# soedinglab/spacedust

Hardware: AMD Instinct MI355X
Metric: clustersearch throughput (genome-pairs/s; SW GCUPS alongside) (higher is better)
Workload: dtype int16

## Files before the change

spacedust_amd/csrc/hip/sd_sw_pk.h:

```cpp
#ifndef SD_SW_PK_H
#define SD_SW_PK_H

#include <hip/hip_runtime.h>
#include <cstdint>

namespace sdpk {

struct SwTask {
    uint64_t qOff;
    uint64_t tOff;
    int32_t n;
    int32_t tL;
    int32_t qStep;
    int32_t tStep;
    int32_t segLen;
    uint32_t slot;
    uint64_t boundOff;
};

typedef short s16x2 __attribute__((ext_vector_type(2)));
typedef unsigned short u16x2 __attribute__((ext_vector_type(2)));

__device__ __forceinline__ uint32_t pkMax(uint32_t a, uint32_t b) {
    return __builtin_bit_cast(uint32_t, __builtin_elementwise_max(__builtin_bit_cast(s16x2, a), __builtin_bit_cast(s16x2, b)));
}
__device__ __forceinline__ uint32_t pkSubSat(uint32_t a, uint32_t b) {
    return __builtin_bit_cast(uint32_t, __builtin_elementwise_sub_sat(__builtin_bit_cast(u16x2, a), __builtin_bit_cast(u16x2, b)));
}
__device__ __forceinline__ uint32_t pkSub(uint32_t a, uint32_t b) {
    return __builtin_bit_cast(uint32_t, (s16x2) (__builtin_bit_cast(s16x2, a) - __builtin_bit_cast(s16x2, b)));
}
__device__ __forceinline__ uint32_t pkAdd(uint32_t a, uint32_t b) {
    return __builtin_bit_cast(uint32_t, (s16x2) (__builtin_bit_cast(s16x2, a) + __builtin_bit_cast(s16x2, b)));
}
__device__ __forceinline__ uint32_t pkLshr(uint32_t a, int s) {
    return __builtin_bit_cast(uint32_t, (u16x2) (__builtin_bit_cast(u16x2, a) >> (u16x2) ((unsigned short) s)));
}
__device__ __forceinline__ uint32_t pkAshr(uint32_t a, int s) {
    return __builtin_bit_cast(uint32_t, (s16x2) (__builtin_bit_cast(s16x2, a) >> (s16x2) ((short) s)));
}
__device__ __forceinline__ uint32_t pkRowCode(uint32_t g, int code) {
    uint32_t r;
    asm("v_pk_mad_i16 %0, %1, 32, %2 op_sel_hi:[1,0,0] clamp" : "=v"(r) : "v"(g), "s"(code));
    return r;
}
__device__ __forceinline__ uint32_t bfi(uint32_t mask, uint32_t a, uint32_t b) { return (a & mask) | (b & ~mask); }

__device__ __forceinline__ void addProfile4(uint32_t pa, uint32_t pb, uint32_t d0, uint32_t d1, uint32_t d2, uint32_t d3,
                                            uint32_t &h0, uint32_t &h1, uint32_t &h2, uint32_t &h3) {
    asm("v_add_u16_sdwa %0, %4, sext(%8) dst_sel:WORD_0 dst_unused:UNUSED_PAD src0_sel:WORD_0 src1_sel:BYTE_0\n\t"
        "v_add_u16_sdwa %1, %5, sext(%8) dst_sel:WORD_0 dst_unused:UNUSED_PAD src0_sel:WORD_0 src1_sel:BYTE_1\n\t"
        "v_add_u16_sdwa %2, %6, sext(%8) dst_sel:WORD_0 dst_unused:UNUSED_PAD src0_sel:WORD_0 src1_sel:BYTE_2\n\t"
        "v_add_u16_sdwa %3, %7, sext(%8) dst_sel:WORD_0 dst_unused:UNUSED_PAD src0_sel:WORD_0 src1_sel:BYTE_3\n\t"
        "v_add_u16_sdwa %0, %4, sext(%9) dst_sel:WORD_1 dst_unused:UNUSED_PRESERVE src0_sel:WORD_1 src1_sel:BYTE_0\n\t"
        "v_add_u16_sdwa %1, %5, sext(%9) dst_sel:WORD_1 dst_unused:UNUSED_PRESERVE src0_sel:WORD_1 src1_sel:BYTE_1\n\t"
        "v_add_u16_sdwa %2, %6, sext(%9) dst_sel:WORD_1 dst_unused:UNUSED_PRESERVE src0_sel:WORD_1 src1_sel:BYTE_2\n\t"
        "v_add_u16_sdwa %3, %7, sext(%9) dst_sel:WORD_1 dst_unused:UNUSED_PRESERVE src0_sel:WORD_1 src1_sel:BYTE_3\n\t"
        "s_nop 0"
        : "=&v"(h0), "=&v"(h1), "=&v"(h2), "=&v"(h3)
        : "v"(d0), "v"(d1), "v"(d2), "v"(d3), "v"(pa), "v"(pb));
}

__device__ __forceinline__ uint32_t dppShr1(uint32_t v) {
    return (uint32_t) __builtin_amdgcn_update_dpp(0, (int) v, 0x138 , 0xf, 0xf, false);
}

template <int LANE>
__device__ __forceinline__ uint32_t writeLane(uint32_t value, uint32_t old) {
    asm("v_writelane_b32 %0, %1, %2" : "+v"(old) : "s"(value), "n"(LANE));
    return old;
}
__device__ __forceinline__ uint32_t readLane(uint32_t v, int lane) {
#if defined(__HIP_DEVICE_COMPILE__)
    return (uint32_t) __builtin_amdgcn_readlane((int) v, lane);
#else
    (void) lane;
    return v;
#endif
}

constexpr int PK_NEUTRAL = 21;

template <int RT, int LW, bool MULTI, bool WIDE, bool SHARED>
__global__ void __launch_bounds__(64)
sw_score_pk_kernel(const SwTask *__restrict__ tasks, uint32_t nTasks, const uint8_t *__restrict__ qRes,
                   const int8_t *__restrict__ qBias, const uint8_t *__restrict__ tRes, const int8_t *__restrict__ mat,
                   int go, int ge, int32_t *__restrict__ out, uint2 *__restrict__ boundary,
                   const uint32_t *__restrict__ order,
                   const int8_t *__restrict__ qProf ) {
    constexpr int ROWS = LW * RT;
    constexpr int WORDS = (RT + 3) / 4;
    constexpr int RTP = 4 * WORDS;
    constexpr int PSTRIDE = LW * WORDS;
    constexpr int NGRP = 64 / LW;
    constexpr int NT = 2 * NGRP;
    __shared__ uint32_t prof[SHARED ? NGRP : NT][22][PSTRIDE];
    __shared__ int8_t smat[441];
    for (int i = threadIdx.x; i < 441; i += 64) smat[i] = mat[i];
    __syncthreads();

    const int lane = threadIdx.x;
    const int grp = lane / LW, l = lane % LW;
    SwTask tk[NT];
#pragma unroll
    for (int x = 0; x < NT; x++) {
        const uint32_t id = blockIdx.x * NT + x;
        const uint32_t tid = id < nTasks ? (order ? order[id] : id) : 0xFFFFFFFFu;
        if (tid != 0xFFFFFFFFu) {
            tk[x] = tasks[tid];
        } else {
            tk[x].n = 0; tk[x].tL = 0; tk[x].qOff = 0; tk[x].tOff = 0; tk[x].qStep = 1; tk[x].tStep = 1; tk[x].segLen = 1;
            tk[x].slot = 0; tk[x].boundOff = 0;
        }
    }
    const SwTask A = (NGRP == 2 && grp) ? tk[NT - 2] : tk[0];
    SwTask B = (NGRP == 2 && grp) ? tk[NT - 1] : tk[1];
    const bool haveA = A.n > 0, haveB = B.n > 0;
    if (SHARED && !haveB) {
        B = A;
        B.tL = 0;
    }
    int maxN = 0, maxTL = 0;
#pragma unroll
    for (int x = 0; x < NT; x++) {
        maxN = max(maxN, tk[x].n);
        maxTL = max(maxTL, tk[x].tL);
    }
    const int pairTL = max(A.tL, B.tL);
    const int nStrips = MULTI ? (maxN + ROWS - 1) / ROWS : (maxN > 0 ? 1 : 0);
    const int steps = (maxN > 0 && maxTL > 0) ? maxTL + LW - 1 : 0;
    uint4 *bnd = nullptr;
    if (MULTI) bnd = (uint4 *) (boundary + (A.tL >= B.tL ? A.boundOff : B.boundOff));

    const uint32_t goP = (uint32_t) go | ((uint32_t) go << 16), geP = (uint32_t) ge | ((uint32_t) ge << 16);
    unsigned long long keyA = 0, keyB = 0;
    const uint32_t *profA = &prof[SHARED ? grp : 2 * grp][0][0] + l * WORDS;
    const uint32_t *profB = SHARED ? profA : &prof[2 * grp + 1][0][0] + l * WORDS;

    for (int strip = 0; strip < nStrips; strip++) {
        const int q0 = strip * ROWS + l * RT;
        uint32_t mask[RTP];
        if (strip > 0) __syncthreads();
#pragma unroll
        for (int x = 0; x < (SHARED ? 1 : 2); x++) {
            const SwTask &T = x ? B : A;
            uint32_t *pw = &prof[SHARED ? grp : 2 * grp + x][0][0] + l * WORDS;
            int seg = T.segLen > 0 ? q0 % T.segLen : 0;
#pragma unroll
            for (int w = 0; w < WORDS; w++) {
                int res[4], cb[4];
                int64_t pidx[4];
                bool valid[4];
#pragma unroll
                for (int b = 0; b < 4; b++) {
                    const int qi = q0 + 4 * w + b;
                    valid[b] = (4 * w + b < RT) && qi < T.n;
                    res[b] = 20;
                    cb[b] = 0;
                    pidx[b] = 0;
                    if (valid[b]) {
                        const int64_t idx = (int64_t) T.qOff + (int64_t) qi * T.qStep;
                        res[b] = qRes[idx];
                        cb[b] = qBias[idx];
                        pidx[b] = idx * 21;
                    }
                    const bool reset = valid[b] && seg == 0;
                    seg = (seg + 1 == T.segLen) ? 0 : seg + 1;
                    const uint32_t m = reset ? 0u : 0xFFFFu;
                    if (SHARED) mask[4 * w + b] = m | (m << 16);
                    else if (x == 0) mask[4 * w + b] = m;
                    else mask[4 * w + b] |= m << 16;
                }
                if (qProf) {
                    for (int a = 0; a < 21; a++) {
                        uint32_t word = 0;
#pragma unroll
                        for (int b = 0; b < 4; b++) {
                            const int v = valid[b] ? (int) qProf[pidx[b] + a] : -64;
                            word |= (uint32_t) (uint8_t) (int8_t) v << (8 * b);
                        }
                        pw[a * PSTRIDE + w] = word;
                    }
                } else {
                    for (int a = 0; a < 21; a++) {
                        uint32_t word = 0;
#pragma unroll
                        for (int b = 0; b < 4; b++) {
                            const int v = valid[b] ? (int) smat[a * 21 + res[b]] + cb[b] : -64;
                            word |= (uint32_t) (uint8_t) (int8_t) v << (8 * b);
                        }
                        pw[a * PSTRIDE + w] = word;
                    }
                }
                pw[PK_NEUTRAL * PSTRIDE + w] = 0xC0C0C0C0u;
            }
        }
        __syncthreads();

        uint32_t H[RTP], E[RTP];
#pragma unroll
        for (int r = 0; r < RTP; r++) {
            H[r] = 0;
            E[r] = 0;
        }
        uint32_t outG = 0, outFf = 0, outFl = 0, prevInG = 0;
        uint32_t curT = PK_NEUTRAL | (PK_NEUTRAL << 8);
        uint32_t bestv = 0, bestcm = 0, bestcol = 0;
        uint32_t bestA = 0, bestB = 0, bcolA = 0, bcolB = 0;
        uint32_t ccol = (uint32_t) (-l) & 0xFFFFu;
        ccol |= ccol << 16;
        const bool lastStrip = strip == nStrips - 1;
        const bool readBound = MULTI && strip > 0;

        auto loadChunk = [&](int c0) -> uint32_t {
            const int col = c0 + l;
            uint32_t a = PK_NEUTRAL, b = PK_NEUTRAL;
            if (col < A.tL) a = tRes[(int64_t) A.tOff + (int64_t) col * A.tStep];
            if (col < B.tL) b = tRes[(int64_t) B.tOff + (int64_t) col * B.tStep];
            return a | (b << 8);
        };
        auto loadBound = [&](int c0) -> uint4 {
            const int col = c0 + l;
            uint4 v = make_uint4(0, 0, 0, 0);
            if (readBound && col < pairTL) {
                const unsigned long long lo = __hip_atomic_load((unsigned long long *) &bnd[col], __ATOMIC_RELAXED, __HIP_MEMORY_SCOPE_AGENT);
                const unsigned long long hi = __hip_atomic_load((unsigned long long *) &bnd[col] + 1, __ATOMIC_RELAXED, __HIP_MEMORY_SCOPE_AGENT);
                v.x = (uint32_t) lo; v.y = (uint32_t) (lo >> 32); v.z = (uint32_t) hi;
            }
            return v;
        };
        if (readBound) __threadfence();

        uint32_t chunk = loadChunk(0);
        uint4 bchunk = loadBound(0);
        for (int k0 = 0; k0 < steps; k0 += LW) {
            const uint32_t chunkNext = loadChunk(k0 + LW);
            uint4 bnext = make_uint4(0, 0, 0, 0);
            if (readBound) bnext = loadBound(k0 + LW);
            const int iEnd = min(LW, steps - k0);
#pragma unroll 1
            for (int i = 0; i < iEnd; i++) {
                uint32_t inT = dppShr1(curT), inG = dppShr1(outG), inFf = dppShr1(outFf), inFl = dppShr1(outFl);
                inT = writeLane<0>(readLane(chunk, i), inT);
                if (NGRP == 2) inT = writeLane<32>(readLane(chunk, 32 + i), inT);
                if (readBound) {
                    inG = writeLane<0>(readLane(bchunk.x, i), inG);
                    inFf = writeLane<0>(readLane(bchunk.y, i), inFf);
                    inFl = writeLane<0>(readLane(bchunk.z, i), inFl);
                    if (NGRP == 2) {
                        inG = writeLane<32>(readLane(bchunk.x, 32 + i), inG);
                        inFf = writeLane<32>(readLane(bchunk.y, 32 + i), inFf);
                        inFl = writeLane<32>(readLane(bchunk.z, 32 + i), inFl);
                    }
                } else if (NGRP == 2) {
                    inG = writeLane<32>(0, inG);
                    inFf = writeLane<32>(0, inFf);
                    inFl = writeLane<32>(0, inFl);
                }
                curT = inT;
                const uint32_t *pa = profA + (curT & 0xFFu) * PSTRIDE;
                const uint32_t *pb = profB + (curT >> 8) * PSTRIDE;
                uint32_t h[RTP];
#pragma unroll
                for (int w = 0; w < WORDS; w++) {
                    const uint32_t d0 = (w == 0) ? prevInG : H[4 * w - 1];
                    addProfile4(pa[w], pb[w], d0, H[4 * w], H[4 * w + 1], H[4 * w + 2], h[4 * w], h[4 * w + 1], h[4 * w + 2],
                                h[4 * w + 3]);
                }
                prevInG = inG;
                uint32_t Fl = inFl, Ff = inFf, cm = 0, cmA = 0, cmB = 0;
#pragma unroll
                for (int r = 0; r < RT; r++) {
                    Fl &= mask[r];
                    const uint32_t hpre = pkMax(pkMax(h[r], E[r]), Fl);
                    const uint32_t g = pkMax(hpre, Ff);
                    const uint32_t open = pkSubSat(hpre, goP);
                    E[r] = pkMax(pkSubSat(E[r], geP), open);
                    Fl = pkMax(pkSubSat(Fl, geP), open);
                    Ff = pkMax(pkSubSat(Ff, geP), open);
                    H[r] = g;
                    if (WIDE) {
                        cmA = max(cmA, (g << 16) | (uint32_t) (31 - r));
                        cmB = max(cmB, (g & 0xFFFF0000u) | (uint32_t) (31 - r));
                    } else {
                        cm = pkMax(cm, pkRowCode(g, 31 - r));
                    }
                }
                outG = H[RT - 1];
                outFf = Ff;
                outFl = Fl;
                if (MULTI && !lastStrip && l == LW - 1) {
                    const int c = k0 + i - (LW - 1);
                    if (c >= 0 && c < pairTL) {
                        const unsigned long long lo = (unsigned long long) outG | ((unsigned long long) outFf << 32);
                        __hip_atomic_store((unsigned long long *) &bnd[c], lo, __ATOMIC_RELAXED, __HIP_MEMORY_SCOPE_AGENT);
                        __hip_atomic_store((unsigned long long *) &bnd[c] + 1, (unsigned long long) outFl, __ATOMIC_RELAXED,
                                           __HIP_MEMORY_SCOPE_AGENT);
                    }
                }
                if (WIDE) {
                    const bool upA = cmA > (bestA | 0xFFFFu), upB = cmB > (bestB | 0xFFFFu);
                    bestA = upA ? cmA : bestA;
                    bcolA = upA ? ccol : bcolA;
                    bestB = upB ? cmB : bestB;
                    bcolB = upB ? ccol : bcolB;
                } else {
                    const uint32_t v = pkLshr(cm, 5);
                    const uint32_t nb = pkMax(bestv, v);
                    const uint32_t m = pkAshr(pkSub(bestv, nb), 15);
                    bestcm = bfi(m, cm, bestcm);
                    bestcol = bfi(m, ccol, bestcol);
                    bestv = nb;
                }
                ccol = pkAdd(ccol, 0x00010001u);
            }
            chunk = chunkNext;
            bchunk = bnext;
        }
        {
            const uint32_t vA = WIDE ? bestA >> 16 : bestv & 0xFFFFu, vB = WIDE ? bestB >> 16 : bestv >> 16;
            const uint32_t rcA = WIDE ? bestA & 31u : bestcm & 31u, rcB = WIDE ? bestB & 31u : (bestcm >> 16) & 31u;
            const uint32_t rowA = (uint32_t) (q0 + 31 - (int) rcA), rowB = (uint32_t) (q0 + 31 - (int) rcB);
            const uint32_t colA = WIDE ? bcolA & 0xFFFFu : bestcol & 0xFFFFu, colB = WIDE ? bcolB >> 16 : bestcol >> 16;
            if (vA > 0) {
                const unsigned long long kk = ((unsigned long long) vA << 40) | ((unsigned long long) (0xFFFFFu - colA) << 20) |
                                              (unsigned long long) (0xFFFFFu - rowA);
                keyA = kk > keyA ? kk : keyA;
            }
            if (vB > 0) {
                const unsigned long long kk = ((unsigned long long) vB << 40) | ((unsigned long long) (0xFFFFFu - colB) << 20) |
                                              (unsigned long long) (0xFFFFFu - rowB);
                keyB = kk > keyB ? kk : keyB;
            }
        }
    }
#pragma unroll
    for (int off = LW / 2; off >= 1; off >>= 1) {
        const unsigned long long oa = __shfl_xor(keyA, off, LW), ob = __shfl_xor(keyB, off, LW);
        keyA = oa > keyA ? oa : keyA;
        keyB = ob > keyB ? ob : keyB;
    }
    if (l == 0) {
        if (haveA) {
            const int v = (int) (keyA >> 40);
            out[3 * A.slot + 0] = v;
            out[3 * A.slot + 1] = v == 0 ? -1 : 0xFFFFF - (int) ((keyA >> 20) & 0xFFFFF);
            out[3 * A.slot + 2] = v == 0 ? A.n - 1 : 0xFFFFF - (int) (keyA & 0xFFFFF);
        }
        if (haveB) {
            const int v = (int) (keyB >> 40);
            out[3 * B.slot + 0] = v;
            out[3 * B.slot + 1] = v == 0 ? -1 : 0xFFFFF - (int) ((keyB >> 20) & 0xFFFFF);
            out[3 * B.slot + 2] = v == 0 ? B.n - 1 : 0xFFFFF - (int) (keyB & 0xFFFFF);
        }
    }
}

__device__ __forceinline__ uint32_t pkAshr15(uint32_t a) {
    uint32_t r;
    asm("v_pk_ashrrev_i16 %0, 15, %1 op_sel_hi:[0,1]" : "=v"(r) : "v"(a));
    return r;
}
__device__ __forceinline__ uint32_t bfiAsm(uint32_t mask, uint32_t a, uint32_t b) {
    uint32_t r;
    asm("v_bfi_b32 %0, %1, %2, %3" : "=v"(r) : "v"(mask), "v"(a), "v"(b));
    return r;
}
__device__ __forceinline__ uint32_t addWord0(uint32_t base, uint32_t packed) {
    uint32_t r;
    asm("v_add_u32_sdwa %0, %1, %2 dst_sel:DWORD dst_unused:UNUSED_PAD src0_sel:DWORD src1_sel:WORD_0" : "=v"(r) : "v"(base), "v"(packed));
    return r;
}
__device__ __forceinline__ uint32_t addWord1(uint32_t base, uint32_t packed) {
    uint32_t r;
    asm("v_add_u32_sdwa %0, %1, %2 dst_sel:DWORD dst_unused:UNUSED_PAD src0_sel:DWORD src1_sel:WORD_1" : "=v"(r) : "v"(base), "v"(packed));
    return r;
}

template <int RT, bool SHARED>
__global__ void __launch_bounds__(64)
sw_score_pk_aligned_kernel(const SwTask *__restrict__ tasks, uint32_t nTasks, const uint8_t *__restrict__ qRes,
                           const int8_t *__restrict__ qBias, const uint8_t *__restrict__ tRes, const int8_t *__restrict__ mat,
                           int go, int ge, int32_t *__restrict__ out, const uint32_t *__restrict__ order,
                           const int8_t *__restrict__ qProf) {
    constexpr int LW = 32;
    constexpr int WORDS = (RT + 3) / 4;
    constexpr int RTP = 4 * WORDS;
    constexpr int PSTRIDE = LW * WORDS;
    constexpr int NGRP = 64 / LW;
    constexpr int NT = 2 * NGRP;
    constexpr uint32_t ROWB = PSTRIDE * 4;
    static_assert(22 * ROWB < 65536, "row offsets travel in 16 bits");
    __shared__ uint32_t prof[SHARED ? 1 : NT][22][PSTRIDE];
    __shared__ int8_t smat[441];
    for (int i = threadIdx.x; i < 441; i += 64) smat[i] = mat[i];
    __syncthreads();
    const int lane = threadIdx.x & 63, wave = threadIdx.x >> 6;
    const int grp = lane / LW, l = lane % LW;
    SwTask tk[NT];
#pragma unroll
    for (int x = 0; x < NT; x++) {
        const uint32_t id = (blockIdx.x + (uint32_t) wave) * NT + x;
        const uint32_t tid = id < nTasks ? (order ? order[id] : id) : 0xFFFFFFFFu;
        if (tid != 0xFFFFFFFFu) {
            tk[x] = tasks[tid];
        } else {
            tk[x].n = 0; tk[x].tL = 0; tk[x].qOff = 0; tk[x].tOff = 0; tk[x].qStep = 1; tk[x].tStep = 1; tk[x].segLen = 1;
            tk[x].slot = 0; tk[x].boundOff = 0;
        }
    }
    SwTask A = tk[0], B = tk[1];
#pragma unroll
    for (int g = 1; g < NGRP; g++)
        if (grp == g) {
            A = tk[2 * g];
            B = tk[2 * g + 1];
        }
    const bool haveA = A.n > 0, haveB = B.n > 0;
    if (SHARED && !haveB) {
        B = A;
        B.tL = 0;
    }
    int maxN = 0, maxTL = 0;
#pragma unroll
    for (int x = 0; x < NT; x++) {
        maxN = max(maxN, tk[x].n);
        maxTL = max(maxTL, tk[x].tL);
    }
    const int steps = (maxN > 0 && maxTL > 0) ? maxTL + LW - 1 : 0;
    const uint32_t goP = (uint32_t) go | ((uint32_t) go << 16), geP = (uint32_t) ge | ((uint32_t) ge << 16);
    const int q0 = l * RT;
#pragma unroll
    for (int x = 0; x < (SHARED ? 1 : 2); x++) {
        const SwTask &T = SHARED ? tk[0] : (x ? B : A);
        uint32_t *pw = &prof[SHARED ? 0 : 2 * grp + x][0][0] + l * WORDS;
#pragma unroll
        for (int w = 0; w < WORDS; w++) {
            int res[4], cb[4];
            int64_t pidx[4];
            bool valid[4];
#pragma unroll
            for (int b = 0; b < 4; b++) {
                const int qi = q0 + 4 * w + b;
                valid[b] = (4 * w + b < RT) && qi < T.n;
                res[b] = 20;
                cb[b] = 0;
                pidx[b] = 0;
                if (valid[b]) {
                    const int64_t idx = (int64_t) T.qOff + (int64_t) qi * T.qStep;
                    res[b] = qRes[idx];
                    cb[b] = qBias[idx];
                    pidx[b] = idx * 21;
                }
            }
            const int aFirst = SHARED ? wave * NGRP + grp : 0, aStep = SHARED ? NGRP : 1;
            if (qProf) {
                for (int a = aFirst; a < 21; a += aStep) {
                    uint32_t word = 0;
#pragma unroll
                    for (int b = 0; b < 4; b++) {
                        const int v = valid[b] ? (int) qProf[pidx[b] + a] : -64;
                        word |= (uint32_t) (uint8_t) (int8_t) v << (8 * b);
                    }
                    pw[a * PSTRIDE + w] = word;
                }
            } else {
                for (int a = aFirst; a < 21; a += aStep) {
                    uint32_t word = 0;
#pragma unroll
                    for (int b = 0; b < 4; b++) {
                        const int v = valid[b] ? (int) smat[a * 21 + res[b]] + cb[b] : -64;
                        word |= (uint32_t) (uint8_t) (int8_t) v << (8 * b);
                    }
                    pw[a * PSTRIDE + w] = word;
                }
            }
            pw[PK_NEUTRAL * PSTRIDE + w] = 0xC0C0C0C0u;
        }
    }
    __syncthreads();
    typedef __attribute__((address_space(3))) uint32_t lds_u32;
    const uint32_t baseA = (uint32_t) (size_t) (lds_u32 *) (&prof[SHARED ? 0 : 2 * grp][0][0] + l * WORDS);
    const uint32_t baseB = SHARED ? baseA : (uint32_t) (size_t) (lds_u32 *) (&prof[2 * grp + 1][0][0] + l * WORDS);
    auto ldsWord = [](uint32_t addr, int w) -> uint32_t { return *((const lds_u32 *) (size_t) addr + w); };

    uint32_t H[RTP], E[RTP];
#pragma unroll
    for (int r = 0; r < RTP; r++) {
        H[r] = 0;
        E[r] = 0;
    }
    uint32_t outG = 0, outFf = 0, prevInG = 0;
    uint32_t bestcm = 0, bestcol = 0;
    constexpr uint32_t NEUT = (uint32_t) PK_NEUTRAL * ROWB;
    auto loadChunk = [&](int c0) -> uint32_t {
        const int col = c0 + l;
        uint32_t a = PK_NEUTRAL, b = PK_NEUTRAL;
        if (col < A.tL) a = tRes[(int64_t) A.tOff + (int64_t) col * A.tStep];
        if (col < B.tL) b = tRes[(int64_t) B.tOff + (int64_t) col * B.tStep];
        return (a * ROWB) | ((b * ROWB) << 16);
    };
    uint32_t chunk = loadChunk(0);
    uint32_t chunkNext = loadChunk(LW);
    uint32_t T = NEUT | (NEUT << 16);
    T = writeLane<0>(readLane(chunk, 0), T);
    T = writeLane<32>(readLane(chunk, 32), T);
    uint32_t pa[WORDS], pb[WORDS];
    {
        const uint32_t aA = addWord0(baseA, T), aB = addWord1(baseB, T);
#pragma unroll
        for (int w = 0; w < WORDS; w++) {
            pa[w] = ldsWord(aA, w);
            pb[w] = ldsWord(aB, w);
        }
    }
    auto columnStep = [&](const int k, const uint32_t &Tc, const uint32_t (&pac)[WORDS], const uint32_t (&pbc)[WORDS], uint32_t &Tn,
                          uint32_t (&pan)[WORDS], uint32_t (&pbn)[WORDS]) {
        const int i1 = (k + 1) & (LW - 1);
        if (i1 == 0) {
            chunk = chunkNext;
            chunkNext = loadChunk(k + 1 + LW);
        }
        Tn = dppShr1(Tc);
        Tn = writeLane<0>(readLane(chunk, i1), Tn);
        Tn = writeLane<32>(readLane(chunk, 32 + i1), Tn);
        {
            const uint32_t aA = addWord0(baseA, Tn), aB = addWord1(baseB, Tn);
#pragma unroll
            for (int w = 0; w < WORDS; w++) {
                pan[w] = ldsWord(aA, w);
                pbn[w] = ldsWord(aB, w);
            }
        }
        uint32_t inG = dppShr1(outG), inFf = dppShr1(outFf);
        inG = writeLane<32>(0, inG);
        inFf = writeLane<32>(0, inFf);
        uint32_t h[RTP];
#pragma unroll
        for (int w = 0; w < WORDS; w++) {
            const uint32_t d0 = (w == 0) ? prevInG : H[4 * w - 1];
            addProfile4(pac[w], pbc[w], d0, H[4 * w], H[4 * w + 1], H[4 * w + 2], h[4 * w], h[4 * w + 1], h[4 * w + 2], h[4 * w + 3]);
        }
        prevInG = inG;
        uint32_t Fl = 0, Ff = inFf, cm = 0;
#pragma unroll
        for (int r = 0; r < RT; r++) {
            uint32_t hpre = pkMax(h[r], E[r]);
            if (r != 0) hpre = pkMax(hpre, Fl);
            const uint32_t g = pkMax(hpre, Ff);
            const uint32_t open = pkSubSat(hpre, goP);
            E[r] = pkMax(pkSubSat(E[r], geP), open);
            if (r == 0) Fl = open;
            else if (r + 1 != RT) Fl = pkMax(pkSubSat(Fl, geP), open);
            Ff = pkMax(pkSubSat(Ff, geP), open);
            H[r] = g;
            const uint32_t code = pkRowCode(g, 31 - r);
            cm = r == 0 ? code : pkMax(cm, code);
        }
        outG = H[RT - 1];
        outFf = Ff;
        const uint32_t t = bestcm | 0x001F001Fu;
        const uint32_t m = pkAshr15(pkSub(t, cm));
        const uint32_t kk = (uint32_t) k | ((uint32_t) k << 16);
        bestcm = bfiAsm(m, cm, bestcm);
        bestcol = bfiAsm(m, kk, bestcol);
    };
    uint32_t T2, pa2[WORDS], pb2[WORDS];
#pragma unroll 1
    for (int k = 0; k < steps; k += 2) {
        columnStep(k, T, pa, pb, T2, pa2, pb2);
        columnStep(k + 1, T2, pa2, pb2, T, pa, pb);
    }
    unsigned long long keyA = 0, keyB = 0;
    {
        const uint32_t vA = (bestcm & 0xFFFFu) >> 5, vB = bestcm >> 21;
        const uint32_t rowA = (uint32_t) (q0 + 31 - (int) (bestcm & 31u)), rowB = (uint32_t) (q0 + 31 - (int) ((bestcm >> 16) & 31u));
        const uint32_t colA = (bestcol & 0xFFFFu) - (uint32_t) l, colB = (bestcol >> 16) - (uint32_t) l;
        if (vA > 0) keyA = ((unsigned long long) vA << 40) | ((unsigned long long) (0xFFFFFu - colA) << 20) | (unsigned long long) (0xFFFFFu - rowA);
        if (vB > 0) keyB = ((unsigned long long) vB << 40) | ((unsigned long long) (0xFFFFFu - colB) << 20) | (unsigned long long) (0xFFFFFu - rowB);
    }
#pragma unroll
    for (int off = LW / 2; off >= 1; off >>= 1) {
        const unsigned long long oa = __shfl_xor(keyA, off, LW), ob = __shfl_xor(keyB, off, LW);
        keyA = oa > keyA ? oa : keyA;
        keyB = ob > keyB ? ob : keyB;
    }
    if (l == 0) {
        if (haveA) {
            const int v = (int) (keyA >> 40);
            out[3 * A.slot + 0] = v;
            out[3 * A.slot + 1] = v == 0 ? -1 : 0xFFFFF - (int) ((keyA >> 20) & 0xFFFFF);
            out[3 * A.slot + 2] = v == 0 ? A.n - 1 : 0xFFFFF - (int) (keyA & 0xFFFFF);
        }
        if (haveB) {
            const int v = (int) (keyB >> 40);
            out[3 * B.slot + 0] = v;
            out[3 * B.slot + 1] = v == 0 ? -1 : 0xFFFFF - (int) ((keyB >> 20) & 0xFFFFF);
            out[3 * B.slot + 2] = v == 0 ? B.n - 1 : 0xFFFFF - (int) (keyB & 0xFFFFF);
        }
    }
}

}
#endif
```

Baseline: 2628.

## Software-pipeline profile LDS loads and restructure F-chain in packed SW kernels

In the general packed kernel, target residues are pre-scaled to LDS byte offsets, and the profile words for the next column are loaded one step ahead. This uses a double-buffered two-step loop with SDWA address adds, replacing the per-column pointer arithmetic and dependent loads. Chunk and boundary reloads are folded into the column step at 32-column boundaries. In the aligned kernel, the far-F chain is rewritten as a decaying carry plus a final max with Fl, which shortens the per-row dependency work. The change adds register pressure from the extra profile buffers and reorders the F recurrence, which could alter results if it is not exactly equivalent.

After: 2671, median of 6. No clear change (+1.6%).

```diff
diff --git a/spacedust_amd/csrc/hip/sd_sw_pk.h b/spacedust_amd/csrc/hip/sd_sw_pk.h
--- a/spacedust_amd/csrc/hip/sd_sw_pk.h
+++ b/spacedust_amd/csrc/hip/sd_sw_pk.h
@@ -79,6 +79,27 @@
 #endif
 }
 
+__device__ __forceinline__ uint32_t pkAshr15(uint32_t a) {
+    uint32_t r;
+    asm("v_pk_ashrrev_i16 %0, 15, %1 op_sel_hi:[0,1]" : "=v"(r) : "v"(a));
+    return r;
+}
+__device__ __forceinline__ uint32_t bfiAsm(uint32_t mask, uint32_t a, uint32_t b) {
+    uint32_t r;
+    asm("v_bfi_b32 %0, %1, %2, %3" : "=v"(r) : "v"(mask), "v"(a), "v"(b));
+    return r;
+}
+__device__ __forceinline__ uint32_t addWord0(uint32_t base, uint32_t packed) {
+    uint32_t r;
+    asm("v_add_u32_sdwa %0, %1, %2 dst_sel:DWORD dst_unused:UNUSED_PAD src0_sel:DWORD src1_sel:WORD_0" : "=v"(r) : "v"(base), "v"(packed));
+    return r;
+}
+__device__ __forceinline__ uint32_t addWord1(uint32_t base, uint32_t packed) {
+    uint32_t r;
+    asm("v_add_u32_sdwa %0, %1, %2 dst_sel:DWORD dst_unused:UNUSED_PAD src0_sel:DWORD src1_sel:WORD_1" : "=v"(r) : "v"(base), "v"(packed));
+    return r;
+}
+
 constexpr int PK_NEUTRAL = 21;
 
 template <int RT, int LW, bool MULTI, bool WIDE, bool SHARED>
@@ -94,6 +115,8 @@
     constexpr int PSTRIDE = LW * WORDS;
     constexpr int NGRP = 64 / LW;
     constexpr int NT = 2 * NGRP;
+    constexpr uint32_t ROWB = PSTRIDE * 4;
+    static_assert(22 * ROWB < 65536, "row offsets travel in 16 bits");
     __shared__ uint32_t prof[SHARED ? NGRP : NT][22][PSTRIDE];
     __shared__ int8_t smat[441];
     for (int i = threadIdx.x; i < 441; i += 64) smat[i] = mat[i];
@@ -134,8 +157,11 @@
 
     const uint32_t goP = (uint32_t) go | ((uint32_t) go << 16), geP = (uint32_t) ge | ((uint32_t) ge << 16);
     unsigned long long keyA = 0, keyB = 0;
-    const uint32_t *profA = &prof[SHARED ? grp : 2 * grp][0][0] + l * WORDS;
-    const uint32_t *profB = SHARED ? profA : &prof[2 * grp + 1][0][0] + l * WORDS;
+    typedef __attribute__((address_space(3))) uint32_t lds_u32;
+    const uint32_t baseA = (uint32_t) (size_t) (lds_u32 *) (&prof[SHARED ? grp : 2 * grp][0][0] + l * WORDS);
+    const uint32_t baseB = SHARED ? baseA : (uint32_t) (size_t) (lds_u32 *) (&prof[2 * grp + 1][0][0] + l * WORDS);
+    auto ldsWord = [](uint32_t addr, int w) -> uint32_t { return *((const lds_u32 *) (size_t) addr + w); };
+    constexpr uint32_t NEUT = (uint32_t) PK_NEUTRAL * ROWB;
 
     for (int strip = 0; strip < nStrips; strip++) {
         const int q0 = strip * ROWS + l * RT;
@@ -204,7 +230,6 @@
             E[r] = 0;
         }
         uint32_t outG = 0, outFf = 0, outFl = 0, prevInG = 0;
-        uint32_t curT = PK_NEUTRAL | (PK_NEUTRAL << 8);
         uint32_t bestv = 0, bestcm = 0, bestcol = 0;
         uint32_t bestA = 0, bestB = 0, bcolA = 0, bcolB = 0;
         uint32_t ccol = (uint32_t) (-l) & 0xFFFFu;
@@ -217,7 +242,7 @@
             uint32_t a = PK_NEUTRAL, b = PK_NEUTRAL;
             if (col < A.tL) a = tRes[(int64_t) A.tOff + (int64_t) col * A.tStep];
             if (col < B.tL) b = tRes[(int64_t) B.tOff + (int64_t) col * B.tStep];
-            return a | (b << 8);
+            return (a * ROWB) | ((b * ROWB) << 16);
         };
         auto loadBound = [&](int c0) -> uint4 {
             const int col = c0 + l;
@@ -232,90 +257,118 @@
         if (readBound) __threadfence();
 
         uint32_t chunk = loadChunk(0);
+        uint32_t chunkNext = loadChunk(LW);
         uint4 bchunk = loadBound(0);
-        for (int k0 = 0; k0 < steps; k0 += LW) {
-            const uint32_t chunkNext = loadChunk(k0 + LW);
-            uint4 bnext = make_uint4(0, 0, 0, 0);
-            if (readBound) bnext = loadBound(k0 + LW);
-            const int iEnd = min(LW, steps - k0);
+        uint4 bnext = make_uint4(0, 0, 0, 0);
+        if (readBound) bnext = loadBound(LW);
+        uint32_t T = NEUT | (NEUT << 16);
+        T = writeLane<0>(readLane(chunk, 0), T);
+        if (NGRP == 2) T = writeLane<32>(readLane(chunk, 32), T);
+        uint32_t pa[WORDS], pb[WORDS];
+        {
+            const uint32_t aA = addWord0(baseA, T), aB = addWord1(baseB, T);
+#pragma unroll
+            for (int w = 0; w < WORDS; w++) {
+                pa[w] = ldsWord(aA, w);
+                pb[w] = ldsWord(aB, w);
+            }
+        }
+        auto columnStep = [&](const int k, const uint32_t &Tc, const uint32_t (&pac)[WORDS], const uint32_t (&pbc)[WORDS], uint32_t &Tn,
+                              uint32_t (&pan)[WORDS], uint32_t (&pbn)[WORDS]) {
+            const int i0 = k & (LW - 1), i1 = (k + 1) & (LW - 1);
+            uint32_t inG = dppShr1(outG), inFf = dppShr1(outFf), inFl = dppShr1(outFl);
+            if (readBound) {
+                inG = writeLane<0>(readLane(bchunk.x, i0), inG);
+                inFf = writeLane<0>(readLane(bchunk.y, i0), inFf);
+                inFl = writeLane<0>(readLane(bchunk.z, i0), inFl);
+                if (NGRP == 2) {
+                    inG = writeLane<32>(readLane(bchunk.x, 32 + i0), inG);
+                    inFf = writeLane<32>(readLane(bchunk.y, 32 + i0), inFf);
+                    inFl = writeLane<32>(readLane(bchunk.z, 32 + i0), inFl);
+                }
+            } else if (NGRP == 2) {
+                inG = writeLane<32>(0, inG);
+                inFf = writeLane<32>(0, inFf);
+                inFl = writeLane<32>(0, inFl);
+            }
+            if (i1 == 0) {
+                chunk = chunkNext;
+                chunkNext = loadChunk(k + 1 + LW);
+                if (readBound) {
+                    bchunk = bnext;
+                    bnext = loadBound(k + 1 + LW);
+                }
+            }
+            Tn = dppShr1(Tc);
+            Tn = writeLane<0>(readLane(chunk, i1), Tn);
+            if (NGRP == 2) Tn = writeLane<32>(readLane(chunk, 32 + i1), Tn);
+            {
+                const uint32_t aA = addWord0(baseA, Tn), aB = addWord1(baseB, Tn);
+#pragma unroll
+                for (int w = 0; w < WORDS; w++) {
+                    pan[w] = ldsWord(aA, w);
+                    pbn[w] = ldsWord(aB, w);
+                }
+            }
+            uint32_t h[RTP];
+#pragma unroll
+            for (int w = 0; w < WORDS; w++) {
+                const uint32_t d0 = (w == 0) ? prevInG : H[4 * w - 1];
+                addProfile4(pac[w], pbc[w], d0, H[4 * w], H[4 * w + 1], H[4 * w + 2], h[4 * w], h[4 * w + 1], h[4 * w + 2],
+                            h[4 * w + 3]);
+            }
+            prevInG = inG;
+            uint32_t Fl = inFl, Ff = inFf, cm = 0, cmA = 0, cmB = 0;
+#pragma unroll
+            for (int r = 0; r < RT; r++) {
+                Fl &= mask[r];
+                const uint32_t hpre = pkMax(pkMax(h[r], E[r]), Fl);
+                const uint32_t g = pkMax(hpre, Ff);
+                const uint32_t open = pkSubSat(hpre, goP);
+                E[r] = pkMax(pkSubSat(E[r], geP), open);
+                Fl = pkMax(pkSubSat(Fl, geP), open);
+                Ff = pkMax(pkSubSat(Ff, geP), open);
+                H[r] = g;
+                if (WIDE) {
+                    cmA = max(cmA, (g << 16) | (uint32_t) (31 - r));
+                    cmB = max(cmB, (g & 0xFFFF0000u) | (uint32_t) (31 - r));
+                } else {
+                    cm = pkMax(cm, pkRowCode(g, 31 - r));
+                }
+            }
+            outG = H[RT - 1];
+            outFf = Ff;
+            outFl = Fl;
+            if (MULTI && !lastStrip && l == LW - 1) {
+                const int c = k - (LW - 1);
+                if (c >= 0 && c < pairTL) {
+                    const unsigned long long lo = (unsigned long long) outG | ((unsigned long long) outFf << 32);
+                    __hip_atomic_store((unsigned long long *) &bnd[c], lo, __ATOMIC_RELAXED, __HIP_MEMORY_SCOPE_AGENT);
+                    __hip_atomic_store((unsigned long long *) &bnd[c] + 1, (unsigned long long) outFl, __ATOMIC_RELAXED,
+                                       __HIP_MEMORY_SCOPE_AGENT);
+                }
+            }
+            if (WIDE) {
+                const bool upA = cmA > (bestA | 0xFFFFu), upB = cmB > (bestB | 0xFFFFu);
+                bestA = upA ? cmA : bestA;
+                bcolA = upA ? ccol : bcolA;
+                bestB = upB ? cmB : bestB;
+                bcolB = upB ? ccol : bcolB;
+            } else {
+                const uint32_t v = pkLshr(cm, 5);
+                const uint32_t nb = pkMax(bestv, v);
+                const uint32_t m = pkAshr(pkSub(bestv, nb), 15);
+                bestcm = bfi(m, cm, bestcm);
+                bestcol = bfi(m, ccol, bestcol);
+                bestv = nb;
+            }
+            ccol = pkAdd(ccol, 0x00010001u);
+        };
+        uint32_t T2, pa2[WORDS], pb2[WORDS];
 #pragma unroll 1
-            for (int i = 0; i < iEnd; i++) {
-                uint32_t inT = dppShr1(curT), inG = dppShr1(outG), inFf = dppShr1(outFf), inFl = dppShr1(outFl);
-                inT = writeLane<0>(readLane(chunk, i), inT);
-                if (NGRP == 2) inT = writeLane<32>(readLane(chunk, 32 + i), inT);
-                if (readBound) {
-                    inG = writeLane<0>(readLane(bchunk.x, i), inG);
-                    inFf = writeLane<0>(readLane(bchunk.y, i), inFf);
-                    inFl = writeLane<0>(readLane(bchunk.z, i), inFl);
-                    if (NGRP == 2) {
-                        inG = writeLane<32>(readLane(bchunk.x, 32 + i), inG);
-                        inFf = writeLane<32>(readLane(bchunk.y, 32 + i), inFf);
-                        inFl = writeLane<32>(readLane(bchunk.z, 32 + i), inFl);
-                    }
-                } else if (NGRP == 2) {
-                    inG = writeLane<32>(0, inG);
-                    inFf = writeLane<32>(0, inFf);
-                    inFl = writeLane<32>(0, inFl);
-                }
-                curT = inT;
-                const uint32_t *pa = profA + (curT & 0xFFu) * PSTRIDE;
-                const uint32_t *pb = profB + (curT >> 8) * PSTRIDE;
-                uint32_t h[RTP];
-#pragma unroll
-                for (int w = 0; w < WORDS; w++) {
-                    const uint32_t d0 = (w == 0) ? prevInG : H[4 * w - 1];
-                    addProfile4(pa[w], pb[w], d0, H[4 * w], H[4 * w + 1], H[4 * w + 2], h[4 * w], h[4 * w + 1], h[4 * w + 2],
-                                h[4 * w + 3]);
-                }
-                prevInG = inG;
-                uint32_t Fl = inFl, Ff = inFf, cm = 0, cmA = 0, cmB = 0;
-#pragma unroll
-                for (int r = 0; r < RT; r++) {
-                    Fl &= mask[r];
-                    const uint32_t hpre = pkMax(pkMax(h[r], E[r]), Fl);
-                    const uint32_t g = pkMax(hpre, Ff);
-                    const uint32_t open = pkSubSat(hpre, goP);
-                    E[r] = pkMax(pkSubSat(E[r], geP), open);
-                    Fl = pkMax(pkSubSat(Fl, geP), open);
-                    Ff = pkMax(pkSubSat(Ff, geP), open);
-                    H[r] = g;
-                    if (WIDE) {
-                        cmA = max(cmA, (g << 16) | (uint32_t) (31 - r));
-                        cmB = max(cmB, (g & 0xFFFF0000u) | (uint32_t) (31 - r));
-                    } else {
-                        cm = pkMax(cm, pkRowCode(g, 31 - r));
-                    }
-                }
-                outG = H[RT - 1];
-                outFf = Ff;
-                outFl = Fl;
-                if (MULTI && !lastStrip && l == LW - 1) {
-                    const int c = k0 + i - (LW - 1);
-                    if (c >= 0 && c < pairTL) {
-                        const unsigned long long lo = (unsigned long long) outG | ((unsigned long long) outFf << 32);
-                        __hip_atomic_store((unsigned long long *) &bnd[c], lo, __ATOMIC_RELAXED, __HIP_MEMORY_SCOPE_AGENT);
-                        __hip_atomic_store((unsigned long long *) &bnd[c] + 1, (unsigned long long) outFl, __ATOMIC_RELAXED,
-                                           __HIP_MEMORY_SCOPE_AGENT);
-                    }
-                }
-                if (WIDE) {
-                    const bool upA = cmA > (bestA | 0xFFFFu), upB = cmB > (bestB | 0xFFFFu);
-                    bestA = upA ? cmA : bestA;
-                    bcolA = upA ? ccol : bcolA;
-                    bestB = upB ? cmB : bestB;
-                    bcolB = upB ? ccol : bcolB;
-                } else {
-                    const uint32_t v = pkLshr(cm, 5);
-                    const uint32_t nb = pkMax(bestv, v);
-                    const uint32_t m = pkAshr(pkSub(bestv, nb), 15);
-                    bestcm = bfi(m, cm, bestcm);
-                    bestcol = bfi(m, ccol, bestcol);
-                    bestv = nb;
-                }
-                ccol = pkAdd(ccol, 0x00010001u);
-            }
-            chunk = chunkNext;
-            bchunk = bnext;
+        for (int k = 0; k < steps; k += 2) {
+            columnStep(k, T, pa, pb, T2, pa2, pb2);
+            columnStep(k + 1, T2, pa2, pb2, T, pa, pb);
         }
         {
             const uint32_t vA = WIDE ? bestA >> 16 : bestv & 0xFFFFu, vB = WIDE ? bestB >> 16 : bestv >> 16;
@@ -354,27 +407,6 @@
             out[3 * B.slot + 2] = v == 0 ? B.n - 1 : 0xFFFFF - (int) (keyB & 0xFFFFF);
         }
     }
-}
-
-__device__ __forceinline__ uint32_t pkAshr15(uint32_t a) {
-    uint32_t r;
-    asm("v_pk_ashrrev_i16 %0, 15, %1 op_sel_hi:[0,1]" : "=v"(r) : "v"(a));
-    return r;
-}
-__device__ __forceinline__ uint32_t bfiAsm(uint32_t mask, uint32_t a, uint32_t b) {
-    uint32_t r;
-    asm("v_bfi_b32 %0, %1, %2, %3" : "=v"(r) : "v"(mask), "v"(a), "v"(b));
-    return r;
-}
-__device__ __forceinline__ uint32_t addWord0(uint32_t base, uint32_t packed) {
-    uint32_t r;
-    asm("v_add_u32_sdwa %0, %1, %2 dst_sel:DWORD dst_unused:UNUSED_PAD src0_sel:DWORD src1_sel:WORD_0" : "=v"(r) : "v"(base), "v"(packed));
-    return r;
-}
-__device__ __forceinline__ uint32_t addWord1(uint32_t base, uint32_t packed) {
-    uint32_t r;
-    asm("v_add_u32_sdwa %0, %1, %2 dst_sel:DWORD dst_unused:UNUSED_PAD src0_sel:DWORD src1_sel:WORD_1" : "=v"(r) : "v"(base), "v"(packed));
-    return r;
 }
 
 template <int RT, bool SHARED>
@@ -542,23 +574,22 @@
             addProfile4(pac[w], pbc[w], d0, H[4 * w], H[4 * w + 1], H[4 * w + 2], h[4 * w], h[4 * w + 1], h[4 * w + 2], h[4 * w + 3]);
         }
         prevInG = inG;
-        uint32_t Fl = 0, Ff = inFf, cm = 0;
+        uint32_t Fl = 0, c = inFf, cm = 0;
 #pragma unroll
         for (int r = 0; r < RT; r++) {
             uint32_t hpre = pkMax(h[r], E[r]);
             if (r != 0) hpre = pkMax(hpre, Fl);
-            const uint32_t g = pkMax(hpre, Ff);
+            const uint32_t g = pkMax(hpre, c);
             const uint32_t open = pkSubSat(hpre, goP);
             E[r] = pkMax(pkSubSat(E[r], geP), open);
-            if (r == 0) Fl = open;
-            else if (r + 1 != RT) Fl = pkMax(pkSubSat(Fl, geP), open);
-            Ff = pkMax(pkSubSat(Ff, geP), open);
+            Fl = r == 0 ? open : pkMax(pkSubSat(Fl, geP), open);
+            c = pkSubSat(c, geP);
             H[r] = g;
             const uint32_t code = pkRowCode(g, 31 - r);
             cm = r == 0 ? code : pkMax(cm, code);
         }
         outG = H[RT - 1];
-        outFf = Ff;
+        outFf = pkMax(c, Fl);
         const uint32_t t = bestcm | 0x001F001Fu;
         const uint32_t m = pkAshr15(pkSub(t, cm));
         const uint32_t kk = (uint32_t) k | ((uint32_t) k << 16);
```
